# MingSun-Tse/Collaborative-Distillation

Measured on AMD Instinct MI355X. Metric: content megapixels/sec, end-to-end 5-level WCT (16x VGG, 4K content, 2K style), higher is better.
Workload: dtype f32 (f16x3 split-MFMA products, fp32 accumulate); 1 GPU; PytorchWCT/WCT.py --mode 16x, 5-level WCT, 3840x2160 content, 2048x2048 style, alpha=1, style-side work included, images resident in HBM; BASELINE configs[1]; content_total=3840x2160, parallelism=content column strips x1

## Files before the change

collaborative-distillation_amd/csrc/conv3x3_sp.hip:

```cpp
#include "wct_common.h"
#include "conv_f16_dev.h"
#include <cstdlib>

namespace {

constexpr int SPH = 16;
constexpr int SP_NPH = FHW * (SPH + 2);
constexpr int SP_NBLK = (SP_NPH + 63) / 64;
constexpr int SP_NPP = SP_NBLK * 64;
constexpr int SP_ACT_DMA = (SP_NPH * 4 + 63) / 64;
__device__ __forceinline__ int sp_slot(int pix, int q) { return pix * 4 + (q ^ ((pix >> 2) & 3)); }

struct SpArgs {
  const char* in;
  char* out;
  const u32x4* wpk;
  const float* bias;
  const float* inv_scale_ptr;
  float inv_scale;
  int H, W, inW, inH;
  int cin, cout, cin_chunks, cout_pad, groups;
  int tiles_x, tiles_y, up_in, relu;
  unsigned* sat;
};

typedef __attribute__((address_space(3))) void* lds_ptr;

#ifdef WCT_SP_TIMING
__device__ unsigned long long g_sp_t[4];
#define SP_STAMP(i) do { if (threadIdx.x == 0) { __builtin_amdgcn_sched_barrier(0); const unsigned long long t_ = __builtin_amdgcn_s_memtime(); \
                         spt[i] += t_ - sptl; sptl = t_; __builtin_amdgcn_sched_barrier(0); } } while (0)
#else
#define SP_STAMP(i)
#endif

template <int CT, bool POOL, bool OUTF32, bool GROUPS>
__global__ __launch_bounds__(512) void conv3x3_sp_kernel(SpArgs a) {
  extern __shared__ __attribute__((aligned(16))) char smem[];
  constexpr int COW = CT * 32;
  constexpr int NWV = 8, CPW = CT;
  constexpr int STAGE16 = 4 * SP_NPP + 36 * COW;
  constexpr int W_DMA = 36 * COW / 64;
  constexpr int W_PER_WAVE = (W_DMA + NWV - 1) / NWV;
  constexpr int SP_ACT_PER_WAVE = (SP_ACT_DMA + NWV - 1) / NWV;
  u32x4* lds = reinterpret_cast<u32x4*>(smem);
  float* biasL = reinterpret_cast<float*>(lds + 2 * STAGE16);
  const int tid = threadIdx.x, lane = tid & 63, wave = __builtin_amdgcn_readfirstlane(tid >> 6);
  const int li = lane & 31, kh = lane >> 5;
  const int rw = wave, c0 = 0;
  const int ntiles = a.tiles_x * a.tiles_y;
  for (int e = tid; e < a.cout_pad; e += NWV * 64) biasL[e] = a.bias[e];
  const float inv = a.inv_scale_ptr ? *a.inv_scale_ptr : a.inv_scale;
  const size_t in_plane = sp16_plane_bytes(a.inH, a.inW);
  unsigned long long satmask = 0ull;
  const float lob = a.relu ? 0.f : -65504.f;

  size_t poff[SP_ACT_PER_WAVE];
  auto tile_offsets = [&](int tile) {
    const int ty0 = (tile / a.tiles_x) * SPH, tx0 = (tile % a.tiles_x) * FTW;
#pragma unroll
    for (int i = 0; i < SP_ACT_PER_WAVE; ++i) {
      int idx = wave + NWV * i;
      idx = idx < SP_ACT_DMA ? idx : SP_ACT_DMA - 1;
      const int slot_pix = idx * 16 + (lane >> 2);
      const int q = (lane & 3) ^ ((slot_pix >> 2) & 3);
      const int pix = slot_pix < SP_NPH ? slot_pix : SP_NPH - 1;
      const int py = pix / FHW, px = pix - py * FHW;
      int gy = reflect_clamp(ty0 - 1 + py, a.H), gx = reflect_clamp(tx0 - 1 + px, a.W);
      if (a.up_in) { gy >>= 1; gx >>= 1; }
      poff[i] = ((size_t)gy * a.inW + gx) * 64 + q * 16;
    }
  };
  auto issue_slice = [&](int i, int ch, int grp, int stage) {
    u32x4* act = lds + stage * STAGE16;
    u32x4* wgt = act + 4 * SP_NPP;
    {
      int idx = wave + NWV * i;
      idx = idx < SP_ACT_DMA ? idx : SP_ACT_DMA - 1;
      __builtin_amdgcn_global_load_lds(a.in + (size_t)ch * in_plane + poff[i], (lds_ptr)(act + idx * 64), 16, 0, 0);
    }
    if (i < W_PER_WAVE) {
      int idx = wave + NWV * i;
      idx = idx < W_DMA ? idx : W_DMA - 1;
      const u32x4* g;
      if constexpr (COW == 64) g = a.wpk + ((size_t)(ch * 36 + idx) * a.cout_pad + grp * 64 + lane);
// ... 41 lines not shown
    if constexpr (OUTF32) {
      if (ok) *reinterpret_cast<f32x4*>(reinterpret_cast<float*>(a.out) + ((size_t)oy * oW + ox) * a.cout + co) = x;
    } else {
#pragma unroll
      for (int k = 0; k < 4; ++k) satmask |= __ballot(x[k] > 65504.f);
      if (!a.relu) {
#pragma unroll
        for (int k = 0; k < 4; ++k) satmask |= __ballot(x[k] < -65504.f);
      }
      const u32x4 w = sp16_pair_exchange_lob(x, lob);
      if (ok) *reinterpret_cast<u32x4*>(a.out + sp16_piece(sp16_plane_bytes(oH, oW), (size_t)oy * oW + ox, co >> 3, kh)) = w;
    }
  };

  f32x16 acc[CPW][2], pend[CPW][2];
  const int xq = ntiles >> 3, xr = ntiles & 7, xcd = blockIdx.x & 7;
  const int tbase = xcd < xr ? xcd * (xq + 1) : xr * (xq + 1) + (xcd - xr) * xq;
  const int ngroups = GROUPS ? a.groups : 1;
  const int nunits = (xq + (xcd < xr ? 1 : 0)) * ngroups, ustep = gridDim.x >> 3;
  int v = blockIdx.x >> 3, ch = 0, stage = 0;
  if (v >= nunits) return;
  int grp = GROUPS ? v % ngroups : 0;
  int tile = tbase + (GROUPS ? v / ngroups : v);
  int dma_tile = tile;
  int pgrp = 0, pty0 = 0, ptx0 = 0;
  bool have_pend = false;
  const unsigned txm = tile_div_magic(a.tiles_x);
  tile_offsets(tile);
#pragma unroll
  for (int i = 0; i < SP_ACT_PER_WAVE; ++i) issue_slice(i, 0, grp, 0);
#ifdef WCT_SP_TIMING
  unsigned long long spt[4] = {0, 0, 0, 0}, sptl = __builtin_amdgcn_s_memtime();
#endif
  while (true) {
    int nv = v, ngrp = grp, nch = ch + 1;
    if (nch == a.cin_chunks) { nch = 0; nv = v + ustep; ngrp = GROUPS ? nv % ngroups : 0; }
    const bool more = nv < nunits;
    asm volatile("s_waitcnt vmcnt(0) lgkmcnt(0)" ::: "memory");
    __builtin_amdgcn_s_barrier();
    asm volatile("" ::: "memory");
    SP_STAMP(0);
    if (more) {
      const int ntile = nv == v ? tile : tbase + (GROUPS ? nv / ngroups : nv);
      if (ntile != dma_tile) { tile_offsets(ntile); dma_tile = ntile; }
    }
    if (ch == 0) {
#pragma unroll
      for (int c = 0; c < CPW; ++c)
#pragma unroll
        for (int p = 0; p < 2; ++p)
#pragma unroll
          for (int r = 0; r < 16; ++r) acc[c][p][r] = 0.f;
    }
    const u32x4* act = lds + stage * STAGE16;
    const u32x4* wgt = act + 4 * SP_NPP;
#pragma unroll
    for (int tap = 0; tap < 9; ++tap) {
      const int dy = tap / 3, dx = tap - dy * 3;
// ... 26 lines not shown
    }
    SP_STAMP(1);
    have_pend = false;
    if (ch + 1 == a.cin_chunks) {
#pragma unroll
      for (int c = 0; c < CPW; ++c)
#pragma unroll
        for (int p = 0; p < 2; ++p) pend[c][p] = acc[c][p];
      int trow_, tcol_;
      tile_rc(tile, a.tiles_x, txm, trow_, tcol_);
      pty0 = trow_ * SPH; ptx0 = tcol_ * FTW; pgrp = grp; have_pend = true;
    }
#ifdef WCT_SP_TIMING
    spt[3] += 1;
#endif
    if (!more) break;
    if (nv != v) { v = nv; tile = dma_tile; }
    grp = ngrp; ch = nch; stage ^= 1;
    SP_STAMP(2);
  }
  if (have_pend) {
#pragma unroll
    for (int k = 0; k < NPIECE; ++k) epilogue_piece(pend, k, pty0, ptx0, pgrp);
  }
  if (satmask != 0ull && lane == 0 && a.sat) sat_raise(a.sat);
#ifdef WCT_SP_TIMING
  SP_STAMP(2);
  if (threadIdx.x == 0) for (int i = 0; i < 4; ++i) atomicAdd(&g_sp_t[i], spt[i]);
#endif
}

template <bool POOL, bool OUTF32>
__global__ __launch_bounds__(512) void conv3x3_sp3_kernel(SpArgs a) {
  extern __shared__ __attribute__((aligned(16))) char smem[];
  constexpr int COW = 32, NWV = 8, CPW = 1, NST = 3;
  constexpr int ACT16 = 4 * SP_NPP;
  constexpr int WCH16 = 36 * COW;
  constexpr int W_DMA = WCH16 / 64;
  constexpr int SP_ACT_PER_WAVE = (SP_ACT_DMA + NWV - 1) / NWV;
// ... 155 lines not shown
      int trow_, tcol_;
      tile_rc(tbase + v, a.tiles_x, txm, trow_, tcol_);
      pty0 = trow_ * SPH; ptx0 = tcol_ * FTW; have_pend = true;
    }
    if (!have1) break;
    v = v1; ch = c1; v1 = v2; c1 = c2; have1 = have2;
    stage = stage == 2 ? 0 : stage + 1;
  }
  if (have_pend) {
#pragma unroll
    for (int k = 0; k < NPIECE; ++k) epilogue_piece(pend, k, pty0, ptx0);
  }
  if (satmask != 0ull && lane == 0 && a.sat) sat_raise(a.sat);
}

template <bool OUTF32>
__global__ __launch_bounds__(512) void conv3x3_sp_up_kernel(SpArgs a) {
  extern __shared__ __attribute__((aligned(16))) char smem[];
  constexpr int COW = 32, NWV = 8;
  constexpr int WSL = 32 * COW;
  constexpr int STAGE16 = 4 * SP_NPP + WSL;
  constexpr int W_DMA = WSL / 64, W_PER_WAVE = W_DMA / NWV;
  constexpr int SP_ACT_PER_WAVE = (SP_ACT_DMA + NWV - 1) / NWV;
  u32x4* lds = reinterpret_cast<u32x4*>(smem);
  float* biasL = reinterpret_cast<float*>(lds + 2 * STAGE16);
  const int tid = threadIdx.x, lane = tid & 63, wave = __builtin_amdgcn_readfirstlane(tid >> 6);
  const int li = lane & 31, kh = lane >> 5, rw = wave;
  const int ntiles = a.tiles_x * a.tiles_y;
  for (int e = tid; e < a.cout_pad; e += NWV * 64) biasL[e] = a.bias[e];
  const float inv = a.inv_scale;
  const size_t in_plane = sp16_plane_bytes(a.inH, a.inW);
// ... 47 lines not shown
    if constexpr (OUTF32) {
      if (ok) *reinterpret_cast<f32x4*>(reinterpret_cast<float*>(a.out) + ((size_t)oy * a.W + ox) * a.cout + co) = x;
    } else {
#pragma unroll
      for (int e = 0; e < 4; ++e) satmask |= __ballot(x[e] > 65504.f);
      if (!a.relu) {
#pragma unroll
        for (int e = 0; e < 4; ++e) satmask |= __ballot(x[e] < -65504.f);
      }
      const u32x4 w = sp16_pair_exchange_lob(x, lob);
      if (ok) *reinterpret_cast<u32x4*>(a.out + sp16_piece(sp16_plane_bytes(a.H, a.W), (size_t)oy * a.W + ox, co >> 3, kh)) = w;
    }
  };

  f32x16 acc[2][2], pend[2][2];
  const int xq = ntiles >> 3, xr = ntiles & 7, xcd = blockIdx.x & 7;
  const int tbase = xcd < xr ? xcd * (xq + 1) : xr * (xq + 1) + (xcd - xr) * xq;
  const int ngroups = a.groups;
  const int nunits = (xq + (xcd < xr ? 1 : 0)) * ngroups, ustep = gridDim.x >> 3;
  int v = blockIdx.x >> 3, ch = 0, stage = 0;
  if (v >= nunits) return;
  int grp = v % ngroups;
  int tile = tbase + v / ngroups;
  int dma_tile = tile;
  int pgrp = 0, pty0 = 0, ptx0 = 0;
  bool have_pend = false;
  const unsigned txm = tile_div_magic(a.tiles_x);
  tile_offsets(tile);
#pragma unroll
  for (int i = 0; i < SP_ACT_PER_WAVE; ++i) issue_slice(i, 0, grp, 0);
  while (true) {
    int nv = v, ngrp = grp, nch = ch + 1;
    if (nch == a.cin_chunks) { nch = 0; nv = v + ustep; ngrp = nv % ngroups; }
    const bool more = nv < nunits;
    asm volatile("s_waitcnt vmcnt(0) lgkmcnt(0)" ::: "memory");
    __builtin_amdgcn_s_barrier();
    asm volatile("" ::: "memory");
    if (more) {
      const int ntile = nv == v ? tile : tbase + nv / ngroups;
      if (ntile != dma_tile) { tile_offsets(ntile); dma_tile = ntile; }
    }
    if (ch == 0) {
#pragma unroll
      for (int b = 0; b < 2; ++b)
#pragma unroll
        for (int p = 0; p < 2; ++p)
#pragma unroll
          for (int r = 0; r < 16; ++r) acc[b][p][r] = 0.f;
    }
    const u32x4* act = lds + stage * STAGE16;
    const u32x4* wgt = act + 4 * SP_NPP;
    const int pa = grp & 1;
#pragma unroll
    for (int it = 0; it < 6; ++it) {
// ... 21 lines not shown
#pragma unroll
          for (int p = 0; p < 2; ++p)
            acc[b][p] = __builtin_amdgcn_mfma_f32_32x32x16_f16(term == 2 ? al : ah, term == 1 ? bl[p] : bh[p], acc[b][p], 0, 0, 0);
      }
    }
    have_pend = false;
    if (ch + 1 == a.cin_chunks) {
#pragma unroll
      for (int b = 0; b < 2; ++b)
#pragma unroll
        for (int p = 0; p < 2; ++p) pend[b][p] = acc[b][p];
      int trow_, tcol_;
      tile_rc(tile, a.tiles_x, txm, trow_, tcol_);
      pty0 = trow_ * SPH; ptx0 = tcol_ * FTW; pgrp = grp; have_pend = true;
    }
    if (!more) break;
    if (nv != v) { v = nv; tile = tbase + nv / ngroups; }
    grp = ngrp; ch = nch; stage ^= 1;
  }
  if (have_pend) {
#pragma unroll
    for (int k = 0; k < NPIECE; ++k) epilogue_piece(pend, k, pty0, ptx0, pgrp);
  }
  if (satmask != 0ull && lane == 0 && a.sat) sat_raise(a.sat);
}

template <typename K>
hipError_t launch_sp(K k, const SpArgs& a, size_t lds, hipStream_t s, int threads, char form = 't') {
  hipError_t e = hipFuncSetAttribute(reinterpret_cast<const void*>(k), hipFuncAttributeMaxDynamicSharedMemorySize, (int)lds);
  if (e != hipSuccess) return e;
  const int ntiles = a.tiles_x * a.tiles_y, want = 8 * ((ntiles + 7) / 8) * a.groups, cus = (num_cus() & ~7) > 8 ? (num_cus() & ~7) : 8;
  const int grid = want < cus ? want : cus;
  note_launch_form(form, SPH, (long)ntiles * a.groups, grid);
  hipLaunchKernelGGL(k, dim3(grid), dim3(threads), lds, s, a);
  return hipGetLastError();
}

}

bool conv_sp_supported(const ConvDesc& d) {
  static const int mask = [] { const char* e = wct_debug_env("WCT_SP_DMA_MASK"); return e ? atoi(e) : 31; }();
  const bool pool = d.flags & CONV_POOL_OUT;
  const int fam = d.cout_pad >= 128 ? 16 : d.cout_pad == 64 ? (pool ? 8 : 4) : (pool ? 2 : 1);
// ... 9 lines not shown
}

hipError_t launch_conv3x3_sp(const ConvDesc& d, const void* in, void* out, int H, int W, hipStream_t s) {
  if (H < 2 || W < 2 || !conv_sp_supported(d) || !(d.flags & CONV_IN_SP16)) return hipErrorInvalidValue;
  SpArgs a;
  a.in = reinterpret_cast<const char*>(in); a.out = reinterpret_cast<char*>(out);
  a.wpk = reinterpret_cast<const u32x4*>(d.wpk16); a.bias = d.bias;
  a.inv_scale_ptr = d.inv_scale_ptr; a.inv_scale = d.inv_scale;
  a.H = H; a.W = W;
  a.up_in = (d.flags & CONV_UP_IN) ? 1 : 0;
  a.inW = a.up_in ? W / 2 : W; a.inH = a.up_in ? H / 2 : H;
  a.cin = d.cin; a.cout = d.cout; a.cin_chunks = d.cin_chunks; a.cout_pad = d.cout_pad;
  a.tiles_x = (W + FTW - 1) / FTW; a.tiles_y = (H + SPH - 1) / SPH;
  a.relu = (d.flags & CONV_NO_RELU) ? 0 : 1;
  a.sat = d.sat;
  const bool pool = d.flags & CONV_POOL_OUT, f32 = !(d.flags & CONV_OUT_SP16);
  if (conv_sp_up_form(d, H, W)) {
    a.wpk = reinterpret_cast<const u32x4*>(d.wup16);
    a.inv_scale = d.inv_scale_up;
    a.tiles_x = (a.inW + FTW - 1) / FTW; a.tiles_y = (a.inH + SPH - 1) / SPH;
    a.groups = 2 * (d.cout_pad / 32);
    const size_t ldsu = (size_t)2 * (4 * SP_NPP + 32 * 32) * 16 + (size_t)d.cout_pad * sizeof(float);
    return f32 ? launch_sp(conv3x3_sp_up_kernel<true>, a, ldsu, s, 512, 'u') : launch_sp(conv3x3_sp_up_kernel<false>, a, ldsu, s, 512, 'u');
  }
  const int ct = (d.cout_pad % 64 == 0) ? 2 : 1;
  a.groups = d.cout_pad / (ct * 32);
  static const int sp3_env = [] { const char* e = wct_debug_env("WCT_SP3"); return e ? atoi(e) : 1; }();
  if (sp3_env && d.cout_pad == 32 && d.cin_chunks <= 2) {
    const size_t lds3 = ((size_t)3 * 4 * SP_NPP + (size_t)d.cin_chunks * 36 * 32) * 16 + (size_t)d.cout_pad * sizeof(float);
    if (pool) return f32 ? launch_sp(conv3x3_sp3_kernel<true, true>, a, lds3, s, 512, '3') : launch_sp(conv3x3_sp3_kernel<true, false>, a, lds3, s, 512, '3');
    return f32 ? launch_sp(conv3x3_sp3_kernel<false, true>, a, lds3, s, 512, '3') : launch_sp(conv3x3_sp3_kernel<false, false>, a, lds3, s, 512, '3');
  }
  const size_t lds = (size_t)2 * (4 * SP_NPP + 36 * ct * 32) * 16 + (size_t)d.cout_pad * sizeof(float);
#define WCT_SP_CASE(CTV, GV)                                                                                          \
  if (ct == CTV && (a.groups > 1) == GV) {                                                                            \
    if (pool) return f32 ? launch_sp(conv3x3_sp_kernel<CTV, true, true, GV>, a, lds, s, 512) : launch_sp(conv3x3_sp_kernel<CTV, true, false, GV>, a, lds, s, 512); \
    return f32 ? launch_sp(conv3x3_sp_kernel<CTV, false, true, GV>, a, lds, s, 512) : launch_sp(conv3x3_sp_kernel<CTV, false, false, GV>, a, lds, s, 512);         \
  }
  WCT_SP_CASE(1, false)
  WCT_SP_CASE(2, false)
  WCT_SP_CASE(2, true)
#undef WCT_SP_CASE
  return hipErrorInvalidValue;
}

#ifdef WCT_SP_TIMING
extern "C" int wct_debug_sp_timing(unsigned long long* out4) {
  unsigned long long z[4] = {0, 0, 0, 0};
  if (hipMemcpyFromSymbol(out4, HIP_SYMBOL(g_sp_t), sizeof(z)) != hipSuccess) return -1;
  return hipMemcpyToSymbol(HIP_SYMBOL(g_sp_t), z, sizeof(z)) == hipSuccess ? 0 : -1;
}
#endif
// ... 1 lines not shown
```

collaborative-distillation_amd/csrc/conv_f16_dev.h:

```cpp
#pragma once
#include "wct_common.h"

namespace {

typedef _Float16 f16x8 __attribute__((ext_vector_type(8)));
typedef float f32x16 __attribute__((ext_vector_type(16)));
typedef unsigned u32x4 __attribute__((ext_vector_type(4)));

constexpr int FTW = 32;
constexpr int FHW = FTW + 2;
constexpr int nph(int TH) { return FHW * (TH + 2); }
constexpr int npp(int TH) { return (nph(TH) + 15) / 16 * 16; }

typedef unsigned u32x2 __attribute__((ext_vector_type(2)));
typedef _Float16 f16x4 __attribute__((ext_vector_type(4)));

__device__ __forceinline__ int reflect_clamp(int i, int n) {
  if (i < 0) i = -i;
  if (i >= n) i = 2 * n - 2 - i;
  i = i < 0 ? 0 : i;
  return i >= n ? n - 1 : i;
}

__device__ __forceinline__ int xcd_swizzle(int bid, int n) {
// ... 406 lines not shown
#pragma unroll
  for (int s = 0; s < 4; ++s) {
    const u32x2 r0 = *reinterpret_cast<const u32x2*>(p + w.off[s][0]), r1 = *reinterpret_cast<const u32x2*>(p + w.off[s][1]);
    const f16x8 b = __builtin_bit_cast(f16x8, u32x4{r0[0], r0[1], r1[0], r1[1]});
    a0 = __builtin_amdgcn_mfma_f32_16x16x32_f16(w.a[0][s], b, a0, 0, 0, 0);
    a1 = __builtin_amdgcn_mfma_f32_16x16x32_f16(w.a[1][s], b, a1, 0, 0, 0);
  }
  x0 = fma4(a0, w.inv, w.bias[0]);
  x1 = fma4(a1, w.inv, w.bias[1]);
  if constexpr (RELU) {
#pragma unroll
    for (int r = 0; r < 4; ++r) { x0[r] = fmaxf(x0[r], 0.f); x1[r] = fmaxf(x1[r], 0.f); }
  }
}

inline int num_cus() {
  static int n = [] {
    int dev = 0, v = 0;
    if (hipGetDevice(&dev) != hipSuccess || hipDeviceGetAttribute(&v, hipDeviceAttributeMultiprocessorCount, dev) != hipSuccess || v < 1) v = 256;
    if (const char* e = wct_debug_env("WCT_CU_RESERVE")) { const int r = atoi(e); if (r > 0 && r < v - 8) v -= r; }
    return v;
  }();
  return n;
}

}
```

collaborative-distillation_amd/csrc/wct_api.hip:

```cpp
#include "../../include/wct_hip.h"
#include "../../include/wct_hip_color.h"
#include "wct_common.h"

#include <cmath>
#include <cstdarg>
#include <cstdlib>
#include <cstdio>
#include <atomic>
#include <cstring>
#include <dlfcn.h>
#include <map>
#include <mutex>
#include <string>
#include <vector>

namespace {

struct DevBuf {
  void* p = nullptr;
  size_t cap = 0;
};

struct LayerDev {
  ConvDesc d{};
// ... 30 lines not shown
  bool side = false;
};

}

__thread LaunchForm wct_launch_form = {0, 0, false};

struct Lane {
  hipStream_t stream = nullptr;
  DevBuf actA, actB, wsMom, wsEig, sums;
  int xcd = 0;
  unsigned* coop = nullptr;
  int coop_epoch = 0;
  unsigned coop_solves = 0;
  bool coop_off = false;
};

struct wct_ctx {
  int device = 0;
  Lane main, side;
  hipEvent_t ev_join = nullptr;
  hipEvent_t ev_smom[6] = {nullptr, nullptr, nullptr, nullptr, nullptr, nullptr};
  hipEvent_t ev_sar[6] = {nullptr, nullptr, nullptr, nullptr, nullptr, nullptr};
  hipEvent_t ev_switch = nullptr;
  hipEvent_t ev_fork = nullptr, ev_style[6] = {nullptr, nullptr, nullptr, nullptr, nullptr, nullptr};
  int eig_skip = 0, eig_calls = 0;
  int foldgemm = 1;
  int nscoop = 1;
  int interleave = 1;
  std::string err;
  Module mod[2][6];
  DevBuf featC, featS, tmpT, wsAsm, small, foldW, foldW16, eigC, eigS[6];
  DevBuf foldS[6];
  bool fold_ready[6] = {false, false, false, false, false, false};
  int cur_level = 0, cur_h = 0, cur_w = 0;
  DevBuf u8c, u8s, u8o;
  DevBuf rsz_tmp;
  std::vector<ResizeAxis> rsz_axes;
  unsigned long long rsz_clock = 0;
  DevBuf noise;
  DevBuf colStyle, colOut, colWs;
  DevBuf l1img;
  int cur_H = 0, cur_W = 0;
// ... 201 lines not shown
      fprintf(tl, "%s %s %.4f %.4f\n", r.name.c_str(), r.side ? "side" : "main", t0, t0 + ms);
    }
    auto& e = ctx->prof_acc[r.name];
    if (e.launches == 0) { memset(&e, 0, sizeof e); snprintf(e.name, sizeof e.name, "%s", r.name.c_str()); }
    e.ms += ms; e.flops += r.flops; e.bytes += r.bytes; e.launches += 1;
  }
  for (auto& r : ctx->recs) { (void)hipEventDestroy(r.e0); (void)hipEventDestroy(r.e1); }
  if (tl) fclose(tl);
  ctx->recs.clear();
}

bool conv_runs_f16(const wct_ctx* ctx, const ConvDesc& d) {
  return ctx->conv_mode == 1 && d.wpk16 && !(d.flags & CONV_IN_NCHW3) && !(d.cin & 7);
}

int run_conv(wct_ctx* ctx, Lane& ln, const ConvDesc& d, const float* in, float* out, int H, int W) {
  char name[48];
  const bool f16 = conv_runs_f16(ctx, d);
  const bool spk = f16 && (d.flags & CONV_IN_SP16) && conv_sp_supported(d);
  if (!f16 && ((d.flags & CONV_IN_SP16) || ((d.flags & CONV_OUT_SP16) && !(d.flags & CONV_IN_NCHW3))))
    return fail(ctx, WCT_ERR_INVALID, "SP16 activations need the f16x3 path");
  snprintf(name, sizeof name, "conv3x3%s<co=%d%s%s%s%s%s>", f16 ? "_f16x3" : "_f32", d.cout_pad > 128 ? 128 : d.cout_pad,
           (d.flags & CONV_IN_NCHW3) ? ",in3" : "", (d.flags & CONV_POOL_OUT) ? ",pool" : "", (d.flags & CONV_OUT_NCHW3) ? ",out3" : "",
           spk ? ",dma" : "", (spk && conv_sp_up_form(d, H, W)) ? ",up" : "");
  static const bool shapes = getenv("WCT_PROF_SHAPES") != nullptr;
  if (shapes) { const size_t n = strlen(name); snprintf(name + n, sizeof name - n, "@%dx%dx%d", H, W, d.cin); }
  const double px = (double)H * W;
  const double in_px = (d.flags & CONV_UP_IN) ? px / 4 : px, out_px = (d.flags & CONV_POOL_OUT) ? px / 4 : px;
  const double flops = 2.0 * 9 * d.cin * d.cout * px;
  const double bytes = 4.0 * (in_px * d.cin + out_px * d.cout + 9.0 * d.cin * d.cout);
  ProfScope ps(ctx, ln.stream, name, flops, bytes);
  if (spk) HIPCHK(ctx, launch_conv3x3_sp(d, in, out, H, W, ln.stream));
  else if (f16) HIPCHK(ctx, launch_conv3x3_f16(d, in, out, H, W, ln.stream));
  else HIPCHK(ctx, launch_conv3x3(d, in, out, H, W, ln.stream));
  return WCT_OK;
}

void pack_weights(const float* w, const float* b, int cout, int cin, int cout_pad, bool in3, const float* c0w,
                  const float* c0b, std::vector<float>& wpk, std::vector<float>& bias) {
  bias.assign(cout_pad, 0.f);
  if (in3) {
    wpk.assign((size_t)36 * cout_pad, 0.f);
    for (int o = 0; o < cout; ++o) {
      double bb = b[o];
      for (int t = 0; t < 9; ++t)
        for (int i = 0; i < 3; ++i) {
          double s = 0.;
// ... 598 lines not shown

int wct_create(int device, wct_ctx** out) {
  if (!out) return WCT_ERR_INVALID;
  *out = nullptr;
  int n = 0;
  if (hipGetDeviceCount(&n) != hipSuccess || device < 0 || device >= n) return WCT_ERR_HIP;
  wct_ctx* c = new (std::nothrow) wct_ctx();
  if (!c) return WCT_ERR_NOMEM;
  c->device = device;
  WCT_GUARD(c);
  if (const char* m = wct_debug_env("WCT_CONV_MODE")) c->conv_mode = (m[0] == '0' || !strcmp(m, "fp32")) ? 0 : 1;
  if (const char* m = wct_debug_env("WCT_OVERLAP")) c->overlap = m[0] != '0';
  if (const char* m = wct_debug_env("WCT_FUSE")) c->fuse = m[0] != '0';
  if (const char* m = wct_debug_env("WCT_SP")) c->sp = m[0] != '0';
  if (const char* m = wct_debug_env("WCT_L1FUSE")) c->l1fuse = m[0] != '0';
  static std::atomic<int> next_xcd{0};
  c->main.xcd = next_xcd.fetch_add(2) & 7;
  c->side.xcd = (c->main.xcd + 1) & 7;
  bool ok = hipStreamCreateWithFlags(&c->side.stream, hipStreamNonBlocking) == hipSuccess;
  for (Lane* ln : {&c->main, &c->side})
    ok = ok && hipMalloc(reinterpret_cast<void**>(&ln->coop), 64) == hipSuccess && hipMemset(ln->coop, 0, 64) == hipSuccess;
  ok = ok && hipEventCreateWithFlags(&c->ev_fork, hipEventDisableTiming) == hipSuccess;
  ok = ok && hipEventCreateWithFlags(&c->ev_join, hipEventDisableTiming) == hipSuccess;
  ok = ok && hipEventCreateWithFlags(&c->ev_switch, hipEventDisableTiming) == hipSuccess;
  for (int l = 1; l <= 5 && ok; ++l)
    ok = hipEventCreateWithFlags(&c->ev_style[l], hipEventDisableTiming) == hipSuccess && hipEventCreateWithFlags(&c->ev_smom[l], hipEventDisableTiming) == hipSuccess &&
         hipEventCreateWithFlags(&c->ev_sar[l], hipEventDisableTiming) == hipSuccess;
  ok = ok && hipMalloc(reinterpret_cast<void**>(&c->sat_dev), 256) == hipSuccess && hipMemset(c->sat_dev, 0, 256) == hipSuccess;
  ok = ok && hipHostMalloc(reinterpret_cast<void**>(&c->sat_host), 64, hipHostMallocDefault) == hipSuccess;
  ok = ok && hipMalloc(reinterpret_cast<void**>(&c->ok_log), 64 * sizeof(int)) == hipSuccess;
  ok = ok && hipHostMalloc(reinterpret_cast<void**>(&c->ok_host), 64 * sizeof(int), hipHostMallocDefault) == hipSuccess;
  if (ok) memset(c->sat_host, 0, 64);
  if (!ok) { wct_destroy(c); return WCT_ERR_HIP; }
  *out = c;
  return WCT_OK;
}

void wct_destroy(wct_ctx* ctx) {
  if (!ctx) return;
  {
  WCT_GUARD(ctx);
  (void)hipStreamSynchronize(ctx->main.stream);
  (void)hipStreamSynchronize(ctx->side.stream);
  prof_collect(ctx);
  for (int k = 0; k < 2; ++k)
    for (int l = 0; l < 6; ++l) free_module(ctx->mod[k][l]);
  ctx->each_buf([](DevBuf& b, Lane*, bool) { release(b); });
  for (Lane* ln : {&ctx->main, &ctx->side}) {
    if (ln->coop) (void)hipFree(ln->coop);
    ln->coop = nullptr;
  }
  for (ResizeAxis& a : ctx->rsz_axes) (void)hipFree(a.bounds);
  ctx->rsz_axes.clear();
  for (int l = 0; l < 6; ++l) {
    if (ctx->ev_style[l]) (void)hipEventDestroy(ctx->ev_style[l]);
    if (ctx->ev_smom[l]) (void)hipEventDestroy(ctx->ev_smom[l]);
    if (ctx->ev_sar[l]) (void)hipEventDestroy(ctx->ev_sar[l]);
  }
  if (ctx->ev_fork) (void)hipEventDestroy(ctx->ev_fork);
  if (ctx->ev_join) (void)hipEventDestroy(ctx->ev_join);
  if (ctx->ev_switch) (void)hipEventDestroy(ctx->ev_switch);
  if (ctx->reg_hist_host) (void)hipHostFree(ctx->reg_hist_host);
  if (ctx->blend_host) (void)hipHostFree(ctx->blend_host);

  if (ctx->side.stream) (void)hipStreamDestroy(ctx->side.stream);
// ... 67 lines not shown
}

int wct_debug_set(wct_ctx* ctx, const char* key, double value) {
  if (!ctx || !key) return WCT_ERR_INVALID;
  WCT_GUARD(ctx);
  const int v = value != 0.0;
  if (!strcmp(key, "fuse")) ctx->fuse = v;
  else if (!strcmp(key, "sp")) ctx->sp = v;
  else if (!strcmp(key, "l1fuse")) ctx->l1fuse = v;
  else if (!strcmp(key, "u8fuse")) ctx->u8fuse = v;
  else if (!strcmp(key, "upconv")) ctx->upconv = v;
  else if (!strcmp(key, "fastfold")) ctx->fastfold = v;
  else if (!strcmp(key, "interleave")) ctx->interleave = v;
  else if (!strcmp(key, "foldgemm")) ctx->foldgemm = v;
  else if (!strcmp(key, "prof_forms")) ctx->prof_forms = v;
  else if (!strcmp(key, "nscoop")) ctx->nscoop = (int)value;
  else if (!strcmp(key, "mom32")) ctx->mom32 = (int)value;
  else if (!strcmp(key, "in3wide")) ctx->in3wide = (int)value;
  else if (!strcmp(key, "poison")) {
    if (value < 0) { ctx->poison = -1; return WCT_OK; }
    if (value > 255 || value != (double)(int)value) return fail(ctx, WCT_ERR_INVALID, "debug_set: 'poison' takes a byte 0..255, or -1 for off");
    ctx->poison = (int)value;
    return poison_scratch(ctx, ctx->poison);
  }
  else if (!strcmp(key, "eig_skip")) {
    if (!getenv("WCT_DEBUG")) return fail(ctx, WCT_ERR_INVALID, "debug_set: 'eig_skip' produces wrong results by design (timing experiment); set WCT_DEBUG to allow it");
    ctx->eig_skip = (int)value; ctx->eig_calls = 0;
  }
  else if (!strcmp(key, "shard_emulate")) {
    if (!getenv("WCT_DEBUG")) return fail(ctx, WCT_ERR_INVALID, "debug_set: 'shard_emulate' produces wrong results by design (timing experiment); set WCT_DEBUG to allow it");
// ... 2 lines not shown
    if (!ctx->coll_set || (ctx->comm_ranks != 1 && !ctx->shard_emulate)) return fail(ctx, WCT_ERR_STATE, "debug_set: 'shard_emulate' needs a ONE-rank communicator on the context");
    if (world < 2 || rank >= world) return fail(ctx, WCT_ERR_INVALID, "debug_set: 'shard_emulate' = 100 * ranks + rank");
    ctx->shard_emulate = true; ctx->comm_ranks = world; ctx->comm_rank = rank;
    return WCT_OK;
  }
  else if (!strcmp(key, "side_priority")) {
    int lo = 0, hi = 0;
    HIPCHK(ctx, hipDeviceGetStreamPriorityRange(&lo, &hi));
    HIPCHK(ctx, hipStreamSynchronize(ctx->side.stream));
    hipStream_t ns = nullptr;
    HIPCHK(ctx, hipStreamCreateWithPriority(&ns, hipStreamNonBlocking, value > 0 ? lo : (value < 0 ? hi : 0)));
    (void)hipStreamDestroy(ctx->side.stream);
    ctx->side.stream = ns;
    return WCT_OK;
  }
  else return fail(ctx, WCT_ERR_INVALID, "debug_set: unknown key '%s' (fuse, sp, l1fuse, u8fuse, upconv, fastfold, interleave, foldgemm, nscoop, in3wide, mom32, eig_skip, side_priority, poison, prof_forms)", key);
  HIPCHK(ctx, hipStreamSynchronize(ctx->side.stream));
  return WCT_OK;
}

int wct_debug_get(wct_ctx* ctx, const char* key, double* value) {
  if (!ctx || !key || !value) return WCT_ERR_INVALID;
  WCT_GUARD(ctx);
  if (!strcmp(key, "nscoop_aborts") || !strcmp(key, "nscoop_solves") || !strcmp(key, "nscoop_off")) {
    if (!strcmp(key, "nscoop_solves")) { *value = (double)ctx->main.coop_solves + (double)ctx->side.coop_solves; return WCT_OK; }
    if (!strcmp(key, "nscoop_off")) { (void)coop_usable(ctx, ctx->main); (void)coop_usable(ctx, ctx->side); *value = (ctx->main.coop_off ? 1 : 0) + (ctx->side.coop_off ? 2 : 0); return WCT_OK; }
    HIPCHK(ctx, hipStreamSynchronize(ctx->side.stream));
    HIPCHK(ctx, hipStreamSynchronize(ctx->main.stream));
    unsigned n[2] = {0u, 0u};
    HIPCHK(ctx, hipMemcpy(n, ctx->sat_dev + 2, sizeof n, hipMemcpyDeviceToHost));
    if (ctx->sat_host) { reinterpret_cast<volatile unsigned*>(ctx->sat_host)[2] = n[0]; reinterpret_cast<volatile unsigned*>(ctx->sat_host)[3] = n[1]; }
    *value = (double)n[0] + (double)n[1];
    return WCT_OK;
  }
  if (!strcmp(key, "ws_allocs")) { *value = (double)ctx->ws_allocs; return WCT_OK; }
  if (!strcmp(key, "ws_bytes")) {
    size_t total = 0;
    ctx->each_buf([&](DevBuf& b, Lane*, bool) { total += b.cap; });
    *value = (double)total;
    return WCT_OK;
  }
  return fail(ctx, WCT_ERR_INVALID, "debug_get: unknown key '%s' (nscoop_aborts, nscoop_solves, nscoop_off, ws_allocs, ws_bytes)", key);
}

int wct_load_module(wct_ctx* ctx, int kind, int level, int n_layers, const wct_layer* layers, const float* c0w,
                    const float* c0b) {
  if (!ctx) return WCT_ERR_INVALID;
  WCT_GUARD(ctx);
  if ((kind != WCT_KIND_ENC && kind != WCT_KIND_DEC) || !valid_level(level) || n_layers < 1 || !layers)
    return fail(ctx, WCT_ERR_INVALID, "load_module: bad kind/level/layers (%d, %d, %d)", kind, level, n_layers);
  for (int i = 0; i < n_layers; ++i) {
    const wct_layer& L = layers[i];
    if (!L.weight || !L.bias || L.cin < 1 || L.cout < 1 || L.cin > 512 || L.cout > 512)
      return fail(ctx, WCT_ERR_INVALID, "load_module: layer %d has bad shape %d->%d or NULL weights", i, L.cin, L.cout);
    if (i > 0 && layers[i - 1].cout != L.cin) return fail(ctx, WCT_ERR_INVALID, "load_module: layer %d cin %d != previous cout %d", i, L.cin, layers[i - 1].cout);
    const bool first = i == 0, last = i == n_layers - 1;
    if (kind == WCT_KIND_ENC && first && L.cin != 3) return fail(ctx, WCT_ERR_INVALID, "encoder must start from 3 channels");
// ... 1443 lines not shown
```

collaborative-distillation_amd/csrc/wct_common.h:

```cpp
#pragma once
#include <hip/hip_runtime.h>
#include <stdint.h>
#include <stddef.h>

#include <stdlib.h>
#include <vector>

typedef float f32x4 __attribute__((ext_vector_type(4)));
typedef double f64x4 __attribute__((ext_vector_type(4)));

static inline const char* wct_debug_env(const char* name) {
  const char* g = getenv("WCT_DEBUG");
  if (!g || !g[0] || (g[0] == '0' && !g[1])) return nullptr;
  return getenv(name);
}

struct LaunchForm { char form; int tile_h; bool multi; };
extern __thread LaunchForm wct_launch_form __attribute__((visibility("hidden")));
static inline void note_launch_form(char form, int tile_h, long units, long grid) {
  wct_launch_form.form = form; wct_launch_form.tile_h = tile_h; wct_launch_form.multi = units > grid;
}

__device__ __forceinline__ void sat_raise(unsigned* counter) {
  const unsigned old = atomicAdd(counter, 1u);
// ... 27 lines not shown
  int cin_chunks;
  int cout_pad;
  int flags;
  const float* wpk;
  const float* bias;
  const void* wpk16 = nullptr;
  float inv_scale = 1.f;
  const float* inv_scale_ptr = nullptr;
  const void* l1w16 = nullptr;
  const float* l1bias = nullptr;
  float l1inv = 1.f;
  const void* wph16 = nullptr;
  const void* wup16 = nullptr;
  float inv_scale_up = 1.f;
  unsigned* sat = nullptr;
};

hipError_t launch_conv3x3(const ConvDesc& d, const float* in, float* out, int H, int W, hipStream_t s);

hipError_t launch_conv3x3_f16(const ConvDesc& d, const float* in, float* out, int H, int W, hipStream_t s);
size_t conv_f16_weight_bytes(int cin, int cout_pad, int taps);
bool conv_sp_supported(const ConvDesc& d);
hipError_t launch_conv3x3_sp(const ConvDesc& d, const void* in, void* out, int H, int W, hipStream_t s);
bool conv_sp_up_form(const ConvDesc& d, int H, int W);
bool conv_fusable_head(const ConvDesc& d0, const ConvDesc& d1);
bool conv_fusable_tail(const ConvDesc& d0, const ConvDesc& d1);
hipError_t launch_enc_head(const ConvDesc& d0, const ConvDesc& d1, const float* img, float* out, int H, int W, hipStream_t s);
hipError_t launch_dec_tail(const ConvDesc& d0, const ConvDesc& d1, const float* in, float* out, int H, int W, hipStream_t s);
bool l1_capable(const ConvDesc& enc0);
bool l1_fusable(const ConvDesc& enc0);
hipError_t launch_l1_encode(const ConvDesc& enc0, const float* img, float* out, int H, int W, hipStream_t s);
// ... 91 lines not shown
```

Before: 1034 MP/s.

## Add atomic work-stealing tile dealer to persistent sp conv kernels

Measured after the change: 1035 MP/s (median of 2 runs). No clear change (+0.1%).

```diff
diff --git a/collaborative-distillation_amd/csrc/conv3x3_sp.hip b/collaborative-distillation_amd/csrc/conv3x3_sp.hip
--- a/collaborative-distillation_amd/csrc/conv3x3_sp.hip
+++ b/collaborative-distillation_amd/csrc/conv3x3_sp.hip
@@ -22,6 +22,8 @@
   int cin, cout, cin_chunks, cout_pad, groups;
   int tiles_x, tiles_y, up_in, relu;
   unsigned* sat;
+  unsigned* deal;
+  int deal_skew_us;
 };
 
 typedef __attribute__((address_space(3))) void* lds_ptr;
@@ -34,7 +36,7 @@
 #define SP_STAMP(i)
 #endif
 
-template <int CT, bool POOL, bool OUTF32, bool GROUPS>
+template <int CT, bool POOL, bool OUTF32, bool GROUPS, bool DEAL>
 __global__ __launch_bounds__(512) void conv3x3_sp_kernel(SpArgs a) {
   extern __shared__ __attribute__((aligned(16))) char smem[];
   constexpr int COW = CT * 32;
@@ -55,7 +57,8 @@
   unsigned long long satmask = 0ull;
   const float lob = a.relu ? 0.f : -65504.f;
 
-  size_t poff[SP_ACT_PER_WAVE];
+  typedef unsigned poff_t;
+  poff_t poff[SP_ACT_PER_WAVE];
   auto tile_offsets = [&](int tile) {
     const int ty0 = (tile / a.tiles_x) * SPH, tx0 = (tile % a.tiles_x) * FTW;
 #pragma unroll
@@ -68,7 +71,7 @@
       const int py = pix / FHW, px = pix - py * FHW;
       int gy = reflect_clamp(ty0 - 1 + py, a.H), gx = reflect_clamp(tx0 - 1 + px, a.W);
       if (a.up_in) { gy >>= 1; gx >>= 1; }
-      poff[i] = ((size_t)gy * a.inW + gx) * 64 + q * 16;
+      poff[i] = ((poff_t)gy * a.inW + gx) * 64 + q * 16;
     }
   };
   auto issue_slice = [&](int i, int ch, int grp, int stage) {
@@ -140,34 +143,55 @@
   };
 
   f32x16 acc[CPW][2], pend[CPW][2];
-  const int xq = ntiles >> 3, xr = ntiles & 7, xcd = blockIdx.x & 7;
-  const int tbase = xcd < xr ? xcd * (xq + 1) : xr * (xq + 1) + (xcd - xr) * xq;
   const int ngroups = GROUPS ? a.groups : 1;
-  const int nunits = (xq + (xcd < xr ? 1 : 0)) * ngroups, ustep = gridDim.x >> 3;
-  int v = blockIdx.x >> 3, ch = 0, stage = 0;
-  if (v >= nunits) return;
-  int grp = GROUPS ? v % ngroups : 0;
-  int tile = tbase + (GROUPS ? v / ngroups : v);
-  int dma_tile = tile;
+  Deal dl;
+  dl.init(a.deal, biasL + a.cout_pad, ntiles, ngroups, DEAL ? a.deal_skew_us : 0);
+  const int xcd = dl.xcd(), ustep = dl.ustep(), uend = dl.qbase(xcd) + dl.qcount(xcd);
+  int v = dl.qbase(xcd) + (blockIdx.x >> 3), ch = 0, stage = 0;
+  if (v >= uend) {
+    if (DEAL && tid == 0) dl.leave();
+    return;
+  }
+  dl.stat = 1;
+  int grp, tile, dma_tile;
   int pgrp = 0, pty0 = 0, ptx0 = 0;
   bool have_pend = false;
   const unsigned txm = tile_div_magic(a.tiles_x);
-  tile_offsets(tile);
-#pragma unroll
-  for (int i = 0; i < SP_ACT_PER_WAVE; ++i) issue_slice(i, 0, grp, 0);
 #ifdef WCT_SP_TIMING
   unsigned long long spt[4] = {0, 0, 0, 0}, sptl = __builtin_amdgcn_s_memtime();
 #endif
+  grp = GROUPS ? v % ngroups : 0;
+  tile = GROUPS ? v / ngroups : v;
+  dma_tile = tile;
+  unsigned tk0 = 0u;
+  if (DEAL && wave == 0) tk0 = dl.request(lane, 2);
+  tile_offsets(tile);
+#pragma unroll
+  for (int i = 0; i < SP_ACT_PER_WAVE; ++i) issue_slice(i, 0, grp, 0);
+  if constexpr (DEAL) {
+    if (wave == 0) dl.resolve(lane, tk0, 2);
+    dl.sent(2);
+  }
   while (true) {
-    int nv = v, ngrp = grp, nch = ch + 1;
-    if (nch == a.cin_chunks) { nch = 0; nv = v + ustep; ngrp = GROUPS ? nv % ngroups : 0; }
-    const bool more = nv < nunits;
     asm volatile("s_waitcnt vmcnt(0) lgkmcnt(0)" ::: "memory");
     __builtin_amdgcn_s_barrier();
     asm volatile("" ::: "memory");
     SP_STAMP(0);
+    int nv = v, ngrp = grp, nch = ch + 1;
+    int ask = -1;
+    unsigned tk = 0u;
+    if constexpr (DEAL) {
+      if (dl.pend()) dl.absorb();
+      if (nch == a.cin_chunks && dl.n1 < 0) dl.need(wave, lane);
+      ask = dl.want();
+      if (ask >= 0 && wave == 0) tk = dl.request(lane, ask);
+    }
+    if (nch == a.cin_chunks) {
+      nch = 0; nv = DEAL ? dl.n1 : (v + ustep < uend ? v + ustep : -1); ngrp = GROUPS ? nv % ngroups : 0;
+    }
+    const bool more = nv >= 0;
     if (more) {
-      const int ntile = nv == v ? tile : tbase + (GROUPS ? nv / ngroups : nv);
+      const int ntile = nv == v ? tile : (GROUPS ? nv / ngroups : nv);
       if (ntile != dma_tile) { tile_offsets(ntile); dma_tile = ntile; }
     }
     if (ch == 0) {
@@ -224,8 +248,14 @@
 #ifdef WCT_SP_TIMING
     spt[3] += 1;
 #endif
+    if constexpr (DEAL) {
+      if (ask >= 0) {
+        if (wave == 0) dl.resolve(lane, tk, ask);
+        dl.sent(ask);
+      }
+    }
     if (!more) break;
-    if (nv != v) { v = nv; tile = dma_tile; }
+    if (nv != v) { v = nv; tile = dma_tile; if (DEAL) (void)dl.pop(); }
     grp = ngrp; ch = nch; stage ^= 1;
     SP_STAMP(2);
   }
@@ -233,6 +263,7 @@
 #pragma unroll
     for (int k = 0; k < NPIECE; ++k) epilogue_piece(pend, k, pty0, ptx0, pgrp);
   }
+  if (DEAL && tid == 0) dl.leave();
   if (satmask != 0ull && lane == 0 && a.sat) sat_raise(a.sat);
 #ifdef WCT_SP_TIMING
   SP_STAMP(2);
@@ -418,7 +449,7 @@
   if (satmask != 0ull && lane == 0 && a.sat) sat_raise(a.sat);
 }
 
-template <bool OUTF32>
+template <bool OUTF32, bool DEAL>
 __global__ __launch_bounds__(512) void conv3x3_sp_up_kernel(SpArgs a) {
   extern __shared__ __attribute__((aligned(16))) char smem[];
   constexpr int COW = 32, NWV = 8;
@@ -496,30 +527,51 @@
   };
 
   f32x16 acc[2][2], pend[2][2];
-  const int xq = ntiles >> 3, xr = ntiles & 7, xcd = blockIdx.x & 7;
-  const int tbase = xcd < xr ? xcd * (xq + 1) : xr * (xq + 1) + (xcd - xr) * xq;
   const int ngroups = a.groups;
-  const int nunits = (xq + (xcd < xr ? 1 : 0)) * ngroups, ustep = gridDim.x >> 3;
-  int v = blockIdx.x >> 3, ch = 0, stage = 0;
-  if (v >= nunits) return;
-  int grp = v % ngroups;
-  int tile = tbase + v / ngroups;
-  int dma_tile = tile;
+  Deal dl;
+  dl.init(a.deal, biasL + a.cout_pad, ntiles, ngroups, DEAL ? a.deal_skew_us : 0);
+  const int xcd = dl.xcd(), ustep = dl.ustep(), uend = dl.qbase(xcd) + dl.qcount(xcd);
+  int v = dl.qbase(xcd) + (blockIdx.x >> 3), ch = 0, stage = 0;
+  if (v >= uend) {
+    if (DEAL && tid == 0) dl.leave();
+    return;
+  }
+  dl.stat = 1;
+  int grp, tile, dma_tile;
   int pgrp = 0, pty0 = 0, ptx0 = 0;
   bool have_pend = false;
   const unsigned txm = tile_div_magic(a.tiles_x);
+  grp = v % ngroups;
+  tile = v / ngroups;
+  dma_tile = tile;
+  unsigned tk0 = 0u;
+  if (DEAL && wave == 0) tk0 = dl.request(lane, 2);
   tile_offsets(tile);
 #pragma unroll
   for (int i = 0; i < SP_ACT_PER_WAVE; ++i) issue_slice(i, 0, grp, 0);
+  if constexpr (DEAL) {
+    if (wave == 0) dl.resolve(lane, tk0, 2);
+    dl.sent(2);
+  }
   while (true) {
-    int nv = v, ngrp = grp, nch = ch + 1;
-    if (nch == a.cin_chunks) { nch = 0; nv = v + ustep; ngrp = nv % ngroups; }
-    const bool more = nv < nunits;
     asm volatile("s_waitcnt vmcnt(0) lgkmcnt(0)" ::: "memory");
     __builtin_amdgcn_s_barrier();
     asm volatile("" ::: "memory");
+    int nv = v, ngrp = grp, nch = ch + 1;
+    int ask = -1;
+    unsigned tk = 0u;
+    if constexpr (DEAL) {
+      if (dl.pend()) dl.absorb();
+      if (nch == a.cin_chunks && dl.n1 < 0) dl.need(wave, lane);
+      ask = dl.want();
+      if (ask >= 0 && wave == 0) tk = dl.request(lane, ask);
+    }
+    if (nch == a.cin_chunks) {
+      nch = 0; nv = DEAL ? dl.n1 : (v + ustep < uend ? v + ustep : -1); ngrp = nv % ngroups;
+    }
+    const bool more = nv >= 0;
     if (more) {
-      const int ntile = nv == v ? tile : tbase + nv / ngroups;
+      const int ntile = nv == v ? tile : nv / ngroups;
       if (ntile != dma_tile) { tile_offsets(ntile); dma_tile = ntile; }
     }
     if (ch == 0) {
@@ -571,19 +623,27 @@
       tile_rc(tile, a.tiles_x, txm, trow_, tcol_);
       pty0 = trow_ * SPH; ptx0 = tcol_ * FTW; pgrp = grp; have_pend = true;
     }
+    if constexpr (DEAL) {
+      if (ask >= 0) {
+        if (wave == 0) dl.resolve(lane, tk, ask);
+        dl.sent(ask);
+      }
+    }
     if (!more) break;
-    if (nv != v) { v = nv; tile = tbase + nv / ngroups; }
+    if (nv != v) { v = nv; tile = nv / ngroups; if (DEAL) (void)dl.pop(); }
     grp = ngrp; ch = nch; stage ^= 1;
   }
   if (have_pend) {
 #pragma unroll
     for (int k = 0; k < NPIECE; ++k) epilogue_piece(pend, k, pty0, ptx0, pgrp);
   }
+  if (DEAL && tid == 0) dl.leave();
   if (satmask != 0ull && lane == 0 && a.sat) sat_raise(a.sat);
 }
 
 template <typename K>
 hipError_t launch_sp(K k, const SpArgs& a, size_t lds, hipStream_t s, int threads, char form = 't') {
+  lds += 16;
   hipError_t e = hipFuncSetAttribute(reinterpret_cast<const void*>(k), hipFuncAttributeMaxDynamicSharedMemorySize, (int)lds);
   if (e != hipSuccess) return e;
   const int ntiles = a.tiles_x * a.tiles_y, want = 8 * ((ntiles + 7) / 8) * a.groups, cus = (num_cus() & ~7) > 8 ? (num_cus() & ~7) : 8;
@@ -623,6 +683,7 @@
   a.tiles_x = (W + FTW - 1) / FTW; a.tiles_y = (H + SPH - 1) / SPH;
   a.relu = (d.flags & CONV_NO_RELU) ? 0 : 1;
   a.sat = d.sat;
+  a.deal = d.deal; a.deal_skew_us = d.deal_skew_us;
   const bool pool = d.flags & CONV_POOL_OUT, f32 = !(d.flags & CONV_OUT_SP16);
   if (conv_sp_up_form(d, H, W)) {
     a.wpk = reinterpret_cast<const u32x4*>(d.wup16);
@@ -630,7 +691,8 @@
     a.tiles_x = (a.inW + FTW - 1) / FTW; a.tiles_y = (a.inH + SPH - 1) / SPH;
     a.groups = 2 * (d.cout_pad / 32);
     const size_t ldsu = (size_t)2 * (4 * SP_NPP + 32 * 32) * 16 + (size_t)d.cout_pad * sizeof(float);
-    return f32 ? launch_sp(conv3x3_sp_up_kernel<true>, a, ldsu, s, 512, 'u') : launch_sp(conv3x3_sp_up_kernel<false>, a, ldsu, s, 512, 'u');
+    if (a.deal) return f32 ? launch_sp(conv3x3_sp_up_kernel<true, true>, a, ldsu, s, 512, 'u') : launch_sp(conv3x3_sp_up_kernel<false, true>, a, ldsu, s, 512, 'u');
+    return f32 ? launch_sp(conv3x3_sp_up_kernel<true, false>, a, ldsu, s, 512, 'u') : launch_sp(conv3x3_sp_up_kernel<false, false>, a, ldsu, s, 512, 'u');
   }
   const int ct = (d.cout_pad % 64 == 0) ? 2 : 1;
   a.groups = d.cout_pad / (ct * 32);
@@ -641,10 +703,15 @@
     return f32 ? launch_sp(conv3x3_sp3_kernel<false, true>, a, lds3, s, 512, '3') : launch_sp(conv3x3_sp3_kernel<false, false>, a, lds3, s, 512, '3');
   }
   const size_t lds = (size_t)2 * (4 * SP_NPP + 36 * ct * 32) * 16 + (size_t)d.cout_pad * sizeof(float);
+  if ((size_t)a.inH * a.inW * 64 > 0xffffffffull) return hipErrorInvalidValue;
 #define WCT_SP_CASE(CTV, GV)                                                                                          \
   if (ct == CTV && (a.groups > 1) == GV) {                                                                            \
-    if (pool) return f32 ? launch_sp(conv3x3_sp_kernel<CTV, true, true, GV>, a, lds, s, 512) : launch_sp(conv3x3_sp_kernel<CTV, true, false, GV>, a, lds, s, 512); \
-    return f32 ? launch_sp(conv3x3_sp_kernel<CTV, false, true, GV>, a, lds, s, 512) : launch_sp(conv3x3_sp_kernel<CTV, false, false, GV>, a, lds, s, 512);         \
+    if (a.deal) {                                                                                                     \
+      if (pool) return f32 ? launch_sp(conv3x3_sp_kernel<CTV, true, true, GV, true>, a, lds, s, 512) : launch_sp(conv3x3_sp_kernel<CTV, true, false, GV, true>, a, lds, s, 512); \
+      return f32 ? launch_sp(conv3x3_sp_kernel<CTV, false, true, GV, true>, a, lds, s, 512) : launch_sp(conv3x3_sp_kernel<CTV, false, false, GV, true>, a, lds, s, 512);         \
+    }                                                                                                                 \
+    if (pool) return f32 ? launch_sp(conv3x3_sp_kernel<CTV, true, true, GV, false>, a, lds, s, 512) : launch_sp(conv3x3_sp_kernel<CTV, true, false, GV, false>, a, lds, s, 512); \
+    return f32 ? launch_sp(conv3x3_sp_kernel<CTV, false, true, GV, false>, a, lds, s, 512) : launch_sp(conv3x3_sp_kernel<CTV, false, false, GV, false>, a, lds, s, 512);         \
   }
   WCT_SP_CASE(1, false)
   WCT_SP_CASE(2, false)
diff --git a/collaborative-distillation_amd/csrc/conv_f16_dev.h b/collaborative-distillation_amd/csrc/conv_f16_dev.h
--- a/collaborative-distillation_amd/csrc/conv_f16_dev.h
+++ b/collaborative-distillation_amd/csrc/conv_f16_dev.h
@@ -444,6 +444,103 @@
   }
 }
 
+typedef __attribute__((address_space(3))) int lds_int;
+struct Deal {
+  unsigned* slot;
+  lds_int* lds;
+  int ntiles, ng;
+  int n1, n2;
+  int st, stat;
+
+  __device__ __forceinline__ int xcd() const { return blockIdx.x & 7; }
+  __device__ __forceinline__ int ustep() const { return gridDim.x >> 3; }
+  __device__ __forceinline__ int sq() const { return st & 15; }
+  __device__ __forceinline__ bool pend() const { return st & 64; }
+  __device__ __forceinline__ int qbase(int y) const {
+    const int xq = ntiles >> 3, xr = ntiles & 7;
+    return (y < xr ? y * (xq + 1) : xr * (xq + 1) + (y - xr) * xq) * ng;
+  }
+  __device__ __forceinline__ int qcount(int y) const { return ((ntiles >> 3) + (y < (ntiles & 7) ? 1 : 0)) * ng; }
+  __device__ __forceinline__ int qrem(int y) const { return qcount(y) - ustep(); }
+
+  __device__ __forceinline__ void init(unsigned* slot_, void* lds_, int ntiles_, int ngroups, int skew_us) {
+    slot = slot_; lds = (lds_int*)lds_; ntiles = ntiles_; ng = ngroups;
+    n1 = n2 = -1; stat = 0;
+    const bool late = skew_us > 0 && xcd() == 0;
+    st = late ? 128 : 0;
+    if (late) {
+      const unsigned long long t0 = wall_clock64(), dt = 100ull * (unsigned)(skew_us < 1000 ? skew_us : 1000);
+      while (wall_clock64() - t0 < dt) __builtin_amdgcn_s_sleep(64);
+    }
+  }
+  __device__ __forceinline__ int pop() { const int u = n1; n1 = n2; n2 = -1; stat += 1; return u; }
+
+  __device__ __forceinline__ int want() const {
+    if (pend() || sq() >= 8) return -1;
+    if (st & 512) return 0;
+    return n1 < 0 ? 2 : (n2 < 0 ? 1 : -1);
+  }
+  __device__ __forceinline__ unsigned request(int lane, int n) const {
+    const int y = (xcd() + sq() + (lane < 8 ? lane : 0)) & 7;
+    unsigned tk = 0u;
+    if (n) {
+      if (lane == 0) tk = __hip_atomic_fetch_add(slot + y * DEAL_LINE, (unsigned)n, __ATOMIC_RELAXED, __HIP_MEMORY_SCOPE_AGENT);
+    } else if (lane >= 1 && lane < 8) tk = __hip_atomic_load(slot + y * DEAL_LINE, __ATOMIC_RELAXED, __HIP_MEMORY_SCOPE_AGENT);
+    return tk;
+  }
+  __device__ __forceinline__ void resolve(int lane, unsigned tk, int n) const {
+    int word;
+    if (n == 0) {
+      const int y = (xcd() + sq() + lane) & 7;
+      const bool live = lane >= 1 && lane < 8 - sq() && (int)tk >= 0 && (int)tk < qrem(y);
+      const unsigned long long m = __ballot(live);
+      word = (int)0x80000000 | (m ? sq() + (int)__builtin_ctzll(m) : 8);
+    } else {
+      const int t = (int)__builtin_amdgcn_readfirstlane(tk);
+      const int y0 = (xcd() + sq()) & 7, got = qrem(y0) - t;
+      word = (t >= 0 && got > 0) ? (qbase(y0) + ustep() + t) | ((n == 2 && got > 1) ? 0x40000000 : 0) : (int)0x80000100;
+    }
+    if (lane == 0) lds[(st >> 4) & 1] = word;
+  }
+  __device__ __forceinline__ void sent(int n) { st = (st & ~512) | 64; (void)n; }
+  __device__ __forceinline__ void absorb() {
+    const int w = __builtin_amdgcn_readfirstlane(lds[(st >> 4) & 1]);
+    st = (st ^ 16) & ~64;
+    if (w >= 0) {
+      const int u = w & 0x3fffffff, k = 1 + ((w >> 30) & 1);
+      if (n1 < 0) { n1 = u; if (k == 2) n2 = u + 1; } else n2 = u;
+      if (sq()) stat += k << 16;
+    } else if (w & 256) st |= 512;
+    else st = (st & ~15) | (w & 15);
+  }
+  __device__ __forceinline__ void need(int wave, int lane) {
+    while (n1 < 0 && sq() < 8) {
+      const int n = (st & 512) ? 0 : 1;
+      if (wave == 0) resolve(lane, request(lane, n), n);
+      sent(n);
+      asm volatile("s_waitcnt lgkmcnt(0)" ::: "memory");
+      __builtin_amdgcn_s_barrier();
+      asm volatile("" ::: "memory");
+      absorb();
+    }
+  }
+  __device__ __forceinline__ void leave() const {
+    if (stat >> 16) __hip_atomic_fetch_add(slot + DEAL_STOLEN, (unsigned)stat >> 16, __ATOMIC_RELAXED, __HIP_MEMORY_SCOPE_AGENT);
+    if ((st & 128) && (stat & 0xffff)) __hip_atomic_fetch_add(slot + DEAL_LATE, (unsigned)stat & 0xffffu, __ATOMIC_RELAXED, __HIP_MEMORY_SCOPE_AGENT);
+    const unsigned mine = __hip_atomic_fetch_add(slot + xcd() * DEAL_LINE + 1, 1u, __ATOMIC_RELAXED, __HIP_MEMORY_SCOPE_AGENT);
+    if (mine != (gridDim.x >> 3) - 1) return;
+    const unsigned out = __hip_atomic_fetch_add(slot + DEAL_EXIT, 1u, __ATOMIC_RELAXED, __HIP_MEMORY_SCOPE_AGENT);
+    if (out == 7) {
+#pragma unroll
+      for (int y = 0; y < 8; ++y) {
+        __hip_atomic_store(slot + y * DEAL_LINE, 0u, __ATOMIC_RELAXED, __HIP_MEMORY_SCOPE_AGENT);
+        __hip_atomic_store(slot + y * DEAL_LINE + 1, 0u, __ATOMIC_RELAXED, __HIP_MEMORY_SCOPE_AGENT);
+      }
+      __hip_atomic_store(slot + DEAL_EXIT, 0u, __ATOMIC_RELAXED, __HIP_MEMORY_SCOPE_AGENT);
+    }
+  }
+};
+
 inline int num_cus() {
   static int n = [] {
     int dev = 0, v = 0;
diff --git a/collaborative-distillation_amd/csrc/wct_api.hip b/collaborative-distillation_amd/csrc/wct_api.hip
--- a/collaborative-distillation_amd/csrc/wct_api.hip
+++ b/collaborative-distillation_amd/csrc/wct_api.hip
@@ -68,6 +68,8 @@
   int coop_epoch = 0;
   unsigned coop_solves = 0;
   bool coop_off = false;
+  unsigned* deal = nullptr;
+  unsigned deal_next = 0;
 };
 
 struct wct_ctx {
@@ -81,6 +83,9 @@
   int eig_skip = 0, eig_calls = 0;
   int foldgemm = 1;
   int nscoop = 1;
+  int deal = 1;
+  int deal_skew_us = 0;
+  double deal_seen[2] = {0.0, 0.0};
   int interleave = 1;
   std::string err;
   Module mod[2][6];
@@ -312,6 +317,11 @@
   return ctx->conv_mode == 1 && d.wpk16 && !(d.flags & CONV_IN_NCHW3) && !(d.cin & 7);
 }
 
+unsigned* deal_slot(wct_ctx* ctx, Lane& ln) {
+  if (!ctx->deal || !ln.deal) return nullptr;
+  return ln.deal + (size_t)(ln.deal_next++ % DEAL_RING) * DEAL_SLOT_WORDS;
+}
+
 int run_conv(wct_ctx* ctx, Lane& ln, const ConvDesc& d, const float* in, float* out, int H, int W) {
   char name[48];
   const bool f16 = conv_runs_f16(ctx, d);
@@ -328,7 +338,11 @@
   const double flops = 2.0 * 9 * d.cin * d.cout * px;
   const double bytes = 4.0 * (in_px * d.cin + out_px * d.cout + 9.0 * d.cin * d.cout);
   ProfScope ps(ctx, ln.stream, name, flops, bytes);
-  if (spk) HIPCHK(ctx, launch_conv3x3_sp(d, in, out, H, W, ln.stream));
+  if (spk) {
+    ConvDesc dd = d;
+    dd.deal = deal_slot(ctx, ln); dd.deal_skew_us = ctx->deal_skew_us;
+    HIPCHK(ctx, launch_conv3x3_sp(dd, in, out, H, W, ln.stream));
+  }
   else if (f16) HIPCHK(ctx, launch_conv3x3_f16(d, in, out, H, W, ln.stream));
   else HIPCHK(ctx, launch_conv3x3(d, in, out, H, W, ln.stream));
   return WCT_OK;
@@ -957,12 +971,15 @@
   if (const char* m = wct_debug_env("WCT_FUSE")) c->fuse = m[0] != '0';
   if (const char* m = wct_debug_env("WCT_SP")) c->sp = m[0] != '0';
   if (const char* m = wct_debug_env("WCT_L1FUSE")) c->l1fuse = m[0] != '0';
+  if (const char* m = wct_debug_env("WCT_DEAL")) c->deal = m[0] != '0';
   static std::atomic<int> next_xcd{0};
   c->main.xcd = next_xcd.fetch_add(2) & 7;
   c->side.xcd = (c->main.xcd + 1) & 7;
   bool ok = hipStreamCreateWithFlags(&c->side.stream, hipStreamNonBlocking) == hipSuccess;
   for (Lane* ln : {&c->main, &c->side})
-    ok = ok && hipMalloc(reinterpret_cast<void**>(&ln->coop), 64) == hipSuccess && hipMemset(ln->coop, 0, 64) == hipSuccess;
+    ok = ok && hipMalloc(reinterpret_cast<void**>(&ln->coop), 64) == hipSuccess && hipMemset(ln->coop, 0, 64) == hipSuccess &&
+         hipMalloc(reinterpret_cast<void**>(&ln->deal), DEAL_RING * DEAL_SLOT_WORDS * sizeof(unsigned)) == hipSuccess &&
+         hipMemset(ln->deal, 0, DEAL_RING * DEAL_SLOT_WORDS * sizeof(unsigned)) == hipSuccess;
   ok = ok && hipEventCreateWithFlags(&c->ev_fork, hipEventDisableTiming) == hipSuccess;
   ok = ok && hipEventCreateWithFlags(&c->ev_join, hipEventDisableTiming) == hipSuccess;
   ok = ok && hipEventCreateWithFlags(&c->ev_switch, hipEventDisableTiming) == hipSuccess;
@@ -992,6 +1009,8 @@
   for (Lane* ln : {&ctx->main, &ctx->side}) {
     if (ln->coop) (void)hipFree(ln->coop);
     ln->coop = nullptr;
+    if (ln->deal) (void)hipFree(ln->deal);
+    ln->deal = nullptr;
   }
   for (ResizeAxis& a : ctx->rsz_axes) (void)hipFree(a.bounds);
   ctx->rsz_axes.clear();
@@ -1089,6 +1108,12 @@
   else if (!strcmp(key, "interleave")) ctx->interleave = v;
   else if (!strcmp(key, "foldgemm")) ctx->foldgemm = v;
   else if (!strcmp(key, "prof_forms")) ctx->prof_forms = v;
+  else if (!strcmp(key, "deal")) ctx->deal = v;
+  else if (!strcmp(key, "deal_skew_us")) {
+    if (!getenv("WCT_DEBUG")) return fail(ctx, WCT_ERR_INVALID, "debug_set: 'deal_skew_us' delays workgroups on purpose (test aid); set WCT_DEBUG to allow it");
+    if (value < 0 || value > 1000) return fail(ctx, WCT_ERR_INVALID, "debug_set: 'deal_skew_us' takes 0..1000 microseconds");
+    ctx->deal_skew_us = (int)value;
+  }
   else if (!strcmp(key, "nscoop")) ctx->nscoop = (int)value;
   else if (!strcmp(key, "mom32")) ctx->mom32 = (int)value;
   else if (!strcmp(key, "in3wide")) ctx->in3wide = (int)value;
@@ -1121,7 +1146,7 @@
     ctx->side.stream = ns;
     return WCT_OK;
   }
-  else return fail(ctx, WCT_ERR_INVALID, "debug_set: unknown key '%s' (fuse, sp, l1fuse, u8fuse, upconv, fastfold, interleave, foldgemm, nscoop, in3wide, mom32, eig_skip, side_priority, poison, prof_forms)", key);
+  else return fail(ctx, WCT_ERR_INVALID, "debug_set: unknown key '%s' (fuse, sp, l1fuse, u8fuse, upconv, fastfold, interleave, foldgemm, nscoop, in3wide, mom32, eig_skip, side_priority, poison, prof_forms, deal, deal_skew_us)", key);
   HIPCHK(ctx, hipStreamSynchronize(ctx->side.stream));
   return WCT_OK;
 }
@@ -1140,6 +1165,21 @@
     *value = (double)n[0] + (double)n[1];
     return WCT_OK;
   }
+  if (!strcmp(key, "deal_stolen") || !strcmp(key, "deal_late_units")) {
+    const int which = !strcmp(key, "deal_stolen") ? 0 : 1;
+    HIPCHK(ctx, hipStreamSynchronize(ctx->side.stream));
+    HIPCHK(ctx, hipStreamSynchronize(ctx->main.stream));
+    double total = 0.0;
+    std::vector<unsigned> ring((size_t)DEAL_RING * DEAL_SLOT_WORDS);
+    for (Lane* ln : {&ctx->main, &ctx->side}) {
+      if (!ln->deal) continue;
+      HIPCHK(ctx, hipMemcpy(ring.data(), ln->deal, ring.size() * sizeof(unsigned), hipMemcpyDeviceToHost));
+      for (int i = 0; i < DEAL_RING; ++i) total += ring[(size_t)i * DEAL_SLOT_WORDS + (which ? DEAL_LATE : DEAL_STOLEN)];
+    }
+    *value = total - ctx->deal_seen[which];
+    ctx->deal_seen[which] = total;
+    return WCT_OK;
+  }
   if (!strcmp(key, "ws_allocs")) { *value = (double)ctx->ws_allocs; return WCT_OK; }
   if (!strcmp(key, "ws_bytes")) {
     size_t total = 0;
@@ -1147,7 +1187,7 @@
     *value = (double)total;
     return WCT_OK;
   }
-  return fail(ctx, WCT_ERR_INVALID, "debug_get: unknown key '%s' (nscoop_aborts, nscoop_solves, nscoop_off, ws_allocs, ws_bytes)", key);
+  return fail(ctx, WCT_ERR_INVALID, "debug_get: unknown key '%s' (nscoop_aborts, nscoop_solves, nscoop_off, ws_allocs, ws_bytes, deal_stolen, deal_late_units)", key);
 }
 
 int wct_load_module(wct_ctx* ctx, int kind, int level, int n_layers, const wct_layer* layers, const float* c0w,
diff --git a/collaborative-distillation_amd/csrc/wct_common.h b/collaborative-distillation_amd/csrc/wct_common.h
--- a/collaborative-distillation_amd/csrc/wct_common.h
+++ b/collaborative-distillation_amd/csrc/wct_common.h
@@ -65,7 +65,12 @@
   const void* wup16 = nullptr;
   float inv_scale_up = 1.f;
   unsigned* sat = nullptr;
+  unsigned* deal = nullptr;
+  int deal_skew_us = 0;
 };
+
+constexpr int DEAL_LINE = 16, DEAL_EXIT = 8 * DEAL_LINE, DEAL_STOLEN = DEAL_EXIT + 2, DEAL_LATE = DEAL_EXIT + 3, DEAL_SLOT_WORDS = 9 * DEAL_LINE,
+              DEAL_RING = 64;
 
 hipError_t launch_conv3x3(const ConvDesc& d, const float* in, float* out, int H, int W, hipStream_t s);
 
```
